# tech-srl/code2vec

Measured on NVIDIA H100. Metric: path-contexts/sec (train step, batch 1024x200), higher is better.
Workload: dtype tf32 operands / fp32 accumulate+storage

## Files before the change

### code2vec_b200/csrc/umma_gemm.cuh

```cuda
#pragma once
#include <cuda.h>
#include <cuda_runtime.h>
#include <limits.h>
#include <stdint.h>

#include "common.cuh"

namespace c2v {
namespace umma {

constexpr int BM = 128;
constexpr int BN = 128;
constexpr int BK = 32;
constexpr int WG_K = 8;
constexpr int STAGES = 4;
constexpr int kThreads = 4 * 128;
constexpr int kRegsProducer = 72;
constexpr int kRegsConsumer = 128;
constexpr int kRegsEpilogue = 184;
static_assert(kRegsProducer + 2 * kRegsConsumer + kRegsEpilogue == 4 * 128, "the roles share the CTA's registers");

__device__ __forceinline__ float fast_tanh(float x) {
  float e, r;
  asm("ex2.approx.ftz.f32 %0, %1;" : "=f"(e) : "f"(x * 2.885390081777927f));
  asm("rcp.approx.ftz.f32 %0, %1;" : "=f"(r) : "f"(e + 1.f));
  return fmaf(-2.f, r, 1.f);
}

__device__ __forceinline__ uint32_t smem_u32(const void* p) { return (uint32_t)__cvta_generic_to_shared(p); }

__device__ __forceinline__ void mbar_init(uint64_t* bar, uint32_t count) {
  asm volatile("mbarrier.init.shared::cta.b64 [%0], %1;" ::"r"(smem_u32(bar)), "r"(count));
}
__device__ __forceinline__ void mbar_expect_tx(uint64_t* bar, uint32_t bytes) {
  asm volatile("mbarrier.expect_tx.relaxed.cta.shared::cta.b64 [%0], %1;" ::"r"(smem_u32(bar)), "r"(bytes) : "memory");
}
__device__ __forceinline__ void mbar_arrive(uint64_t* bar) {
  asm volatile("mbarrier.arrive.shared::cta.b64 _, [%0];" ::"r"(smem_u32(bar)) : "memory");
}
__device__ __forceinline__ void mbar_arrive_expect_tx(uint64_t* bar, uint32_t bytes) {
  asm volatile("mbarrier.arrive.expect_tx.shared::cta.b64 _, [%0], %1;" ::"r"(smem_u32(bar)), "r"(bytes) : "memory");
}
__device__ __forceinline__ bool mbar_try_wait(uint64_t* bar, uint32_t parity) {
  uint32_t ok;
  asm volatile(
      "{\n\t.reg .pred p;\n\t"
      "mbarrier.try_wait.parity.shared::cta.b64 p, [%1], %2;\n\t"
      "selp.u32 %0, 1, 0, p;\n\t}"
      : "=r"(ok) : "r"(smem_u32(bar)), "r"(parity) : "memory");
  return ok != 0;
}
template <bool SLEEP = false>
__device__ __forceinline__ void mbar_wait(uint64_t* bar, uint32_t parity) {
  if (mbar_try_wait(bar, parity)) return;
  const long long t0 = clock64();
  uint32_t ns = 32;
  while (!mbar_try_wait(bar, parity)) {
    if (SLEEP) {
      __nanosleep(ns);
      if (ns < 256) ns *= 2;
    }
    if (clock64() - t0 > 20000000000LL) __trap();
  }
}
__device__ __forceinline__ void fence_proxy_async_smem() { asm volatile("fence.proxy.async.shared::cta;" ::: "memory"); }

__device__ __forceinline__ void tma_load_2d(void* smem_dst, const CUtensorMap* map, uint64_t* bar, int c0, int c1) {
  asm volatile(
      "cp.async.bulk.tensor.2d.shared::cluster.global.mbarrier::complete_tx::bytes [%0], [%1, {%3, %4}], [%2];"
      ::"r"(smem_u32(smem_dst)), "l"(map), "r"(smem_u32(bar)), "r"(c0), "r"(c1) : "memory");
}

__device__ __forceinline__ uint64_t gmma_desc(uint32_t saddr) {
  return (uint64_t)((saddr >> 4) & 0x3FFF) | (1ull << 16) | ((uint64_t)(1024 >> 4) << 32) | (1ull << 62);
}
__device__ __forceinline__ void wg_fence() { asm volatile("wgmma.fence.sync.aligned;" ::: "memory"); }
__device__ __forceinline__ void wg_commit() { asm volatile("wgmma.commit_group.sync.aligned;" ::: "memory"); }
template <int N>
__device__ __forceinline__ void wg_wait() { asm volatile("wgmma.wait_group.sync.aligned %0;" ::"n"(N) : "memory"); }
template <int R>
__device__ __forceinline__ void wg_regs_dec() { asm volatile("setmaxnreg.dec.sync.aligned.u32 %0;" ::"n"(R)); }
template <int R>
__device__ __forceinline__ void wg_regs_inc() { asm volatile("setmaxnreg.inc.sync.aligned.u32 %0;" ::"n"(R)); }
__device__ __forceinline__ void wgmma_tf32(float (&d)[64], uint64_t da, uint64_t db, uint32_t accumulate) {
  asm volatile(
      "{\n\t.reg .pred p;\n\t"
      "setp.ne.b32 p, %66, 0;\n\t"
      "wgmma.mma_async.sync.aligned.m64n128k8.f32.tf32.tf32 "
      "{%0, %1, %2, %3, %4, %5, %6, %7, %8, %9, %10, %11, %12, %13, %14, %15, %16, %17, %18, %19, %20, %21, %22, %23, "
      "%24, %25, %26, %27, %28, %29, %30, %31, %32, %33, %34, %35, %36, %37, %38, %39, %40, %41, %42, %43, %44, %45, "
      "%46, %47, %48, %49, %50, %51, %52, %53, %54, %55, %56, %57, %58, %59, %60, %61, %62, %63}, %64, %65, p, 1, 1;\n\t}"
      : "+f"(d[0]), "+f"(d[1]), "+f"(d[2]), "+f"(d[3]), "+f"(d[4]), "+f"(d[5]), "+f"(d[6]), "+f"(d[7]), "+f"(d[8]),
        "+f"(d[9]), "+f"(d[10]), "+f"(d[11]), "+f"(d[12]), "+f"(d[13]), "+f"(d[14]), "+f"(d[15]), "+f"(d[16]),
        "+f"(d[17]), "+f"(d[18]), "+f"(d[19]), "+f"(d[20]), "+f"(d[21]), "+f"(d[22]), "+f"(d[23]), "+f"(d[24]),
        "+f"(d[25]), "+f"(d[26]), "+f"(d[27]), "+f"(d[28]), "+f"(d[29]), "+f"(d[30]), "+f"(d[31]), "+f"(d[32]),
        "+f"(d[33]), "+f"(d[34]), "+f"(d[35]), "+f"(d[36]), "+f"(d[37]), "+f"(d[38]), "+f"(d[39]), "+f"(d[40]),
        "+f"(d[41]), "+f"(d[42]), "+f"(d[43]), "+f"(d[44]), "+f"(d[45]), "+f"(d[46]), "+f"(d[47]), "+f"(d[48]),
        "+f"(d[49]), "+f"(d[50]), "+f"(d[51]), "+f"(d[52]), "+f"(d[53]), "+f"(d[54]), "+f"(d[55]), "+f"(d[56]),
        "+f"(d[57]), "+f"(d[58]), "+f"(d[59]), "+f"(d[60]), "+f"(d[61]), "+f"(d[62]), "+f"(d[63])
      : "l"(da), "l"(db), "r"(accumulate));
}

struct EpiNoState {};

struct EpiStore {
  using State = EpiNoState;
  float* C;
  size_t ldc;
  size_t split_stride;
  __device__ __forceinline__ void begin(State&) const {}
  __device__ __forceinline__ void end(int, int, int, bool, State&) const {}
  __device__ __forceinline__ void observe(int, int, const uint32_t (&)[32], int, State&) const {}
  __device__ __forceinline__ float map(float x) const { return x; }
  __device__ __forceinline__ float* out(int split) const { return C + (size_t)split * split_stride; }
  using Pre = EpiNoState;
  static constexpr int kRowBatch = 8;
  static constexpr bool kMoveRegs = false;
  __device__ __forceinline__ void prefetch(const float*, size_t, Pre&) const {}
  __device__ __forceinline__ void store4(float* c, size_t off, float4 v, const Pre&) const { *reinterpret_cast<float4*>(c + off) = v; }
  __device__ __forceinline__ void store1(float* c, size_t off, float x) const { c[off] = x; }
};
template <bool PRECISE>
struct EpiTanhStoreT {
  using State = EpiNoState;
  float* C;
  size_t ldc;
  __device__ __forceinline__ void begin(State&) const {}
  __device__ __forceinline__ void end(int, int, int, bool, State&) const {}
  __device__ __forceinline__ void observe(int, int, const uint32_t (&)[32], int, State&) const {}
  __device__ __forceinline__ float map(float x) const { return PRECISE ? tanhf(x) : fast_tanh(x); }
  __device__ __forceinline__ float* out(int) const { return C; }
  using Pre = EpiNoState;
  static constexpr int kRowBatch = 8;
  __device__ __forceinline__ void prefetch(const float*, size_t, Pre&) const {}
  __device__ __forceinline__ void store4(float* c, size_t off, float4 v, const Pre&) const { *reinterpret_cast<float4*>(c + off) = v; }
  __device__ __forceinline__ void store1(float* c, size_t off, float x) const { c[off] = x; }
};

template <bool PRECISE>
struct EpiStoreLseT {
  struct State { float mx, sum; };
  float* C;
  size_t ldc;
  float2* partial;
  int slots;
  __device__ __forceinline__ float ex(float x) const { return PRECISE ? expf(x) : __expf(x); }
  __device__ __forceinline__ void begin(State& st) const { st.mx = -INFINITY; st.sum = 0.f; }
  __device__ __forceinline__ void end(int m, int slot, int, bool row_ok, State& st) const {
    if (row_ok) partial[(size_t)m * slots + slot] = make_float2(st.mx, st.sum);
  }
  __device__ __forceinline__ float map(float x) const { return x; }
  __device__ __forceinline__ float* out(int) const { return C; }
  using Pre = EpiNoState;
  static constexpr int kRowBatch = 8;
  __device__ __forceinline__ void prefetch(const float*, size_t, Pre&) const {}
  __device__ __forceinline__ void store4(float* c, size_t off, float4 v, const Pre&) const { *reinterpret_cast<float4*>(c + off) = v; }
  __device__ __forceinline__ void store1(float* c, size_t off, float x) const { c[off] = x; }
  __device__ __forceinline__ void observe(int, int, const uint32_t (&r)[32], int nvalid, State& st) const {
    float cm = -INFINITY;
    if (nvalid >= 32) {
#pragma unroll
      for (int j = 0; j < 32; ++j) cm = fmaxf(cm, __uint_as_float(r[j]));
    } else {
#pragma unroll
      for (int j = 0; j < 32; ++j)
        if (j < nvalid) cm = fmaxf(cm, __uint_as_float(r[j]));
    }
    if (cm > st.mx) { st.sum *= ex(st.mx - cm); st.mx = cm; }
    float a0 = 0.f, a1 = 0.f, a2 = 0.f, a3 = 0.f;
    if (!PRECISE && nvalid >= 32) {
      constexpr float L2E = 1.4426950408889634f;
      const float c = -st.mx * L2E;
      auto e2 = [](float t) { float y; asm("ex2.approx.ftz.f32 %0, %1;" : "=f"(y) : "f"(t)); return y; };
#pragma unroll
      for (int j = 0; j < 32; j += 4) {
        a0 += e2(fmaf(__uint_as_float(r[j + 0]), L2E, c));
        a1 += e2(fmaf(__uint_as_float(r[j + 1]), L2E, c));
        a2 += e2(fmaf(__uint_as_float(r[j + 2]), L2E, c));
        a3 += e2(fmaf(__uint_as_float(r[j + 3]), L2E, c));
      }
    } else {
#pragma unroll
      for (int j = 0; j < 32; j += 4) {
        if (j + 0 < nvalid) a0 += ex(__uint_as_float(r[j + 0]) - st.mx);
        if (j + 1 < nvalid) a1 += ex(__uint_as_float(r[j + 1]) - st.mx);
        if (j + 2 < nvalid) a2 += ex(__uint_as_float(r[j + 2]) - st.mx);
        if (j + 3 < nvalid) a3 += ex(__uint_as_float(r[j + 3]) - st.mx);
      }
    }
    st.sum += (a0 + a1) + (a2 + a3);
  }
};

template <bool PRECISE>
struct EpiLseOnlyT : EpiStoreLseT<PRECISE> {
  static constexpr bool kStores = false;
};
constexpr int kTopkEpiMax = 16;
template <bool PRECISE, bool LSE>
struct EpiTopkT : EpiStoreLseT<PRECISE> {
  using Lse = EpiStoreLseT<PRECISE>;
  struct State {
    float v[kTopkEpiMax];
    int i[kTopkEpiMax];
    typename Lse::State ls;
  };
  float* cand_val;
  int32_t* cand_idx;
  int k;
  int row0;
  static constexpr bool kStores = false;
  __device__ __forceinline__ void begin(State& st) const {
#pragma unroll
    for (int q = 0; q < kTopkEpiMax; ++q) {
      st.v[q] = q < kTopkEpiMax - k ? INFINITY : -INFINITY;
      st.i[q] = INT_MAX;
    }
    if (LSE) Lse::begin(st.ls);
  }
  __device__ __forceinline__ void insert(float x, int col, State& st) const {
#pragma unroll
    for (int q = kTopkEpiMax - 1; q > 0; --q) {
      const bool here = x > st.v[q], above = x > st.v[q - 1];
      st.v[q] = above ? st.v[q - 1] : (here ? x : st.v[q]);
      st.i[q] = above ? st.i[q - 1] : (here ? col : st.i[q]);
    }
    if (x > st.v[0]) { st.v[0] = x; st.i[0] = col; }
  }
  __device__ __forceinline__ void observe(int m, int n, const uint32_t (&r)[32], int nvalid, State& st) const {
    if (LSE) Lse::observe(m, n, r, nvalid, st.ls);
    const float kth = st.v[kTopkEpiMax - 1];
    float x[32];
    uint32_t todo = 0;
#pragma unroll
    for (int j = 0; j < 32; ++j) {
      x[j] = __uint_as_float(r[j]);
      if (j < nvalid && x[j] > kth) todo |= 1u << j;
    }
#pragma unroll 1
    while (todo) {
      const int j = __ffs(todo) - 1;
      todo &= todo - 1;
      insert(x[j], n + j, st);
    }
  }
  __device__ __forceinline__ void end(int m, int slot, int sp, bool row_ok, State& st) const {
    if (!row_ok) return;
    if (LSE) Lse::end(m, slot, sp, row_ok, st.ls);
    const size_t base = ((size_t)m * this->slots + slot) * k;
#pragma unroll
    for (int q = 0; q < kTopkEpiMax; ++q) {
      const int p = q - (kTopkEpiMax - k);
      if (p >= 0) {
        cand_val[base + p] = st.v[q];
        cand_idx[base + p] = st.i[q] == INT_MAX ? INT_MAX : st.i[q] + row0;
      }
    }
  }
};
template <bool PRECISE, bool SPLIT>
struct EpiSoftmaxGradT {
  struct State { float l; int tgt; };
  float* C;
  float* C_lo;
  size_t ldc;
  const float* lse;
  const int32_t* target;
  int row0;
  float inv_batch;
  int M;
  __device__ __forceinline__ void begin(State& st) const { st.l = 0.f; st.tgt = -1; }
  __device__ __forceinline__ void end(int, int, int, bool, State&) const {}
  __device__ __forceinline__ void observe(int m, int, const uint32_t (&)[32], int, State& st) const {
    st.l = PRECISE ? lse[m] : fmaf(-lse[m], 1.4426950408889634f, log2f(inv_batch));
    st.tgt = target[m] - row0;
  }
  __device__ __forceinline__ float map(float x) const { return x; }
  __device__ __forceinline__ float map_at(float x, int col, const State& st) const {
    float p;
    if (PRECISE) {
      p = expf(x - st.l) * inv_batch;
    } else {
      asm("ex2.approx.ftz.f32 %0, %1;" : "=f"(p) : "f"(fmaf(x, 1.4426950408889634f, st.l)));
    }
    return col == st.tgt ? p - inv_batch : p;
  }
  __device__ __forceinline__ float* out(int) const { return C; }
  using Pre = EpiNoState;
  static constexpr int kRowBatch = 8;
  __device__ __forceinline__ void prefetch(const float*, size_t, Pre&) const {}
  __device__ __forceinline__ void store4(float* c, size_t off, float4 v, const Pre&) const {
    if (SPLIT) {
      float4 hi, lo;
      split_tf32(v, hi, lo);
      *reinterpret_cast<float4*>(c + off) = hi;
      *reinterpret_cast<float4*>(C_lo + off) = lo;
    } else {
      *reinterpret_cast<float4*>(c + off) = v;
    }
  }
  __device__ __forceinline__ void store1(float* c, size_t off, float x) const {
    if (SPLIT) {
      float hi, lo;
      split_tf32(x, hi, lo);
      c[off] = hi; C_lo[off] = lo;
    } else {
      c[off] = x;
    }
  }
};

template <bool PRECISE, bool SPLIT>
struct EpiExpSumT {
  struct State { float mx, sum; };
  float* C;
  float* C_lo;
  size_t ldc;
  const float* offset;
  float2* partial;
  int slots;
  __device__ __forceinline__ void begin(State& st) const { st.mx = 0.f; st.sum = 0.f; }
  __device__ __forceinline__ void end(int m, int slot, int, bool row_ok, State& st) const {
    if (row_ok) partial[(size_t)m * slots + slot] = make_float2(st.mx, st.sum);
  }
  __device__ __forceinline__ float map(float x) const { return x; }
  __device__ __forceinline__ float* out(int) const { return C; }
  using Pre = EpiNoState;
  static constexpr int kRowBatch = 8;
  __device__ __forceinline__ void prefetch(const float*, size_t, Pre&) const {}
  __device__ __forceinline__ void store4(float* c, size_t off, float4 v, const Pre&) const {
    if (SPLIT) {
      float4 hi, lo;
      split_tf32(v, hi, lo);
      *reinterpret_cast<float4*>(c + off) = hi;
      *reinterpret_cast<float4*>(C_lo + off) = lo;
    } else {
      *reinterpret_cast<float4*>(c + off) = v;
    }
  }
  __device__ __forceinline__ void store1(float* c, size_t off, float x) const {
    if (SPLIT) {
      float hi, lo;
      split_tf32(x, hi, lo);
      c[off] = hi; C_lo[off] = lo;
    } else {
      c[off] = x;
    }
  }
  __device__ __forceinline__ void observe(int m, int, uint32_t (&r)[32], int nvalid, State& st) const {
    const float c = offset[m];
    float a0 = 0.f, a1 = 0.f, a2 = 0.f, a3 = 0.f, x0 = 0.f, x1 = 0.f, x2 = 0.f, x3 = 0.f;
    if (!PRECISE && nvalid >= 32) {
      constexpr float L2E = 1.4426950408889634f;
      const float c2 = -c * L2E;
      auto e2 = [](float t) { float y; asm("ex2.approx.ftz.f32 %0, %1;" : "=f"(y) : "f"(t)); return y; };
#pragma unroll
      for (int j = 0; j < 32; j += 4) {
        const float u0 = e2(fmaf(__uint_as_float(r[j + 0]), L2E, c2)), u1 = e2(fmaf(__uint_as_float(r[j + 1]), L2E, c2));
        const float u2 = e2(fmaf(__uint_as_float(r[j + 2]), L2E, c2)), u3 = e2(fmaf(__uint_as_float(r[j + 3]), L2E, c2));
        r[j + 0] = __float_as_uint(u0); r[j + 1] = __float_as_uint(u1); r[j + 2] = __float_as_uint(u2); r[j + 3] = __float_as_uint(u3);
        a0 += u0; a1 += u1; a2 += u2; a3 += u3;
        x0 = fmaxf(x0, u0); x1 = fmaxf(x1, u1); x2 = fmaxf(x2, u2); x3 = fmaxf(x3, u3);
      }
    } else {
#pragma unroll
      for (int j = 0; j < 32; ++j) {
        float u = 0.f;
        if (j < nvalid) u = PRECISE ? expf(__uint_as_float(r[j]) - c) : __expf(__uint_as_float(r[j]) - c);
        r[j] = __float_as_uint(u);
        if ((j & 3) == 0) { a0 += u; x0 = fmaxf(x0, u); }
        else if ((j & 3) == 1) { a1 += u; x1 = fmaxf(x1, u); }
        else if ((j & 3) == 2) { a2 += u; x2 = fmaxf(x2, u); }
        else { a3 += u; x3 = fmaxf(x3, u); }
      }
    }
    st.sum += (a0 + a1) + (a2 + a3);
    st.mx = fmaxf(st.mx, fmaxf(fmaxf(x0, x1), fmaxf(x2, x3)));
  }
};
template <bool PRECISE>
struct EpiStoreLseGatedT : EpiStoreLseT<PRECISE> {
  const int* gate;
};

using EpiTanhStore = EpiTanhStoreT<false>;
using EpiTanhStorePrecise = EpiTanhStoreT<true>;
using EpiStoreLse = EpiStoreLseT<false>;
using EpiStoreLsePrecise = EpiStoreLseT<true>;

struct EpiAdam {
  using State = EpiNoState;
  float* P;
  float* Mo;
  float* Vo;
  size_t ldc;
  float lr_t, b1, b2, eps, omb1, omb2;
  int l2_prefetch;
  __device__ __forceinline__ void begin(State&) const {}
  __device__ __forceinline__ void end(int, int, int, bool, State&) const {}
  __device__ __forceinline__ void observe(int, int, const uint32_t (&)[32], int, State&) const {}
  __device__ __forceinline__ float map(float x) const { return x; }
  __device__ __forceinline__ float* out(int) const { return P; }
  __device__ __forceinline__ void upd(float& pp, float gg, float& mm, float& vv) const {
    mm = __fadd_rn(__fmul_rn(mm, b1), __fmul_rn(omb1, gg));
    vv = __fadd_rn(__fmul_rn(vv, b2), __fmul_rn(omb2, __fmul_rn(gg, gg)));
    pp = adam_move_dense(pp, lr_t, mm, vv, eps);
  }
  __device__ __forceinline__ void prefetch_tile(int m, int n0, int ncols, int M, int N) const {
    if (m >= M || !l2_prefetch) return;
    const size_t row = (size_t)m * ldc;
    for (int n = n0; n < n0 + ncols && n < N; n += 32) {
      asm volatile("prefetch.global.L2 [%0];" ::"l"(P + row + n));
      asm volatile("prefetch.global.L2 [%0];" ::"l"(Mo + row + n));
      asm volatile("prefetch.global.L2 [%0];" ::"l"(Vo + row + n));
    }
  }
  struct Pre { float4 p, m, v; };
  static constexpr int kRowBatch = 4;
  __device__ __forceinline__ void prefetch(const float* c, size_t off, Pre& q) const {
    q.p = *reinterpret_cast<const float4*>(c + off);
    q.m = *reinterpret_cast<const float4*>(Mo + off);
    q.v = *reinterpret_cast<const float4*>(Vo + off);
  }
  __device__ __forceinline__ void store4(float* c, size_t off, float4 g, const Pre& q) const {
    float4 p = q.p, m = q.m, v = q.v;
    upd(p.x, g.x, m.x, v.x); upd(p.y, g.y, m.y, v.y); upd(p.z, g.z, m.z, v.z); upd(p.w, g.w, m.w, v.w);
    *reinterpret_cast<float4*>(c + off) = p;
    *reinterpret_cast<float4*>(Mo + off) = m;
    *reinterpret_cast<float4*>(Vo + off) = v;
  }
  __device__ __forceinline__ void store1(float* c, size_t off, float g) const {
    float p = c[off], m = Mo[off], v = Vo[off];
    upd(p, g, m, v);
    c[off] = p; Mo[off] = m; Vo[off] = v;
  }
};

template <class Epi>
__device__ __forceinline__ auto epi_map(const Epi& epi, float x, int col, const typename Epi::State& st, int)
    -> decltype(epi.map_at(x, col, st)) {
  return epi.map_at(x, col, st);
}
template <class Epi>
__device__ __forceinline__ float epi_map(const Epi& epi, float x, int, const typename Epi::State&, long) {
  return epi.map(x);
}
template <class Epi>
__device__ __forceinline__ auto epi_gate_closed(const Epi& epi, int) -> decltype(*epi.gate == 0) { return *epi.gate == 0; }
template <class Epi>
__device__ __forceinline__ bool epi_gate_closed(const Epi&, long) { return false; }
template <class Epi>
__device__ __forceinline__ auto epi_prefetch_tile(const Epi& epi, int m, int n0, int ncols, int M, int N, int)
    -> decltype(epi.prefetch_tile(m, n0, ncols, M, N)) {
  epi.prefetch_tile(m, n0, ncols, M, N);
}
template <class Epi>
__device__ __forceinline__ void epi_prefetch_tile(const Epi&, int, int, int, int, int, long) {}
template <class Epi>
constexpr bool epi_move_regs(...) { return true; }
template <class Epi, bool V = Epi::kMoveRegs>
constexpr bool epi_move_regs(int) { return V; }
template <class Epi>
constexpr bool epi_stores(...) { return true; }
template <class Epi, bool V = Epi::kStores>
constexpr bool epi_stores(int) { return V; }

template <class Epi>
__device__ __forceinline__ void store_chunk(const Epi& epi, const typename Epi::State& est, const uint32_t (&r)[32], float* stage, int lane,
                                            int m_base, int n, int M, int N, float* cbase, size_t ldc) {
#pragma unroll
  for (int j4 = 0; j4 < 8; ++j4) {
    const int pos = j4 ^ (lane & 7);
    *reinterpret_cast<float4*>(stage + lane * 32 + pos * 4) =
        make_float4(epi_map(epi, __uint_as_float(r[4 * j4]), n + 4 * j4, est, 0), epi_map(epi, __uint_as_float(r[4 * j4 + 1]), n + 4 * j4 + 1, est, 0),
                    epi_map(epi, __uint_as_float(r[4 * j4 + 2]), n + 4 * j4 + 2, est, 0), epi_map(epi, __uint_as_float(r[4 * j4 + 3]), n + 4 * j4 + 3, est, 0));
  }
  __syncwarp();
  const int col4 = lane & 7;
  const int gn = n + col4 * 4;
  constexpr int kBatch = Epi::kRowBatch;
  static_assert(8 % kBatch == 0, "the batches tile the chunk's 8 row groups: a remainder would reach into the next block");
#pragma unroll
  for (int it0 = 0; it0 < 8; it0 += kBatch) {
    float4 v[kBatch];
    typename Epi::Pre pre[kBatch];
#pragma unroll
    for (int i = 0; i < kBatch; ++i) {
      const int row = (it0 + i) * 4 + (lane >> 3);
      v[i] = *reinterpret_cast<const float4*>(stage + row * 32 + ((col4 ^ (row & 7)) * 4));
      const int gm = m_base + row;
      if (gm < M && gn + 3 < N) epi.prefetch(cbase, (size_t)gm * ldc + gn, pre[i]);
    }
#pragma unroll
    for (int i = 0; i < kBatch; ++i) {
      const int gm = m_base + (it0 + i) * 4 + (lane >> 3);
      if (gm < M && gn < N) {
        const size_t off = (size_t)gm * ldc + gn;
        if (gn + 3 < N) {
          epi.store4(cbase, off, v[i], pre[i]);
        } else {
          epi.store1(cbase, off, v[i].x);
          if (gn + 1 < N) epi.store1(cbase, off + 1, v[i].y);
          if (gn + 2 < N) epi.store1(cbase, off + 2, v[i].z);
        }
      }
    }
  }
  __syncwarp();
}

struct AXNone {
  static constexpr int kKind = 0;
};

struct SoftmaxGradArgs {
  const float* lse;
  const int32_t* target;
  int row0;
  float inv_batch;
};
__device__ __forceinline__ float ex2_approx(float x) {
  float y;
  asm("ex2.approx.ftz.f32 %0, %1;" : "=f"(y) : "f"(x));
  return y;
}
constexpr float kLog2e = 1.4426950408889634f;

template <bool EX_IS_M>
struct AXSoftmaxGrad {
  static constexpr int kKind = 1;
  SoftmaxGradArgs a;
  __device__ __forceinline__ void example(int ex, float& c, int& tgt) const {
    c = fmaf(-a.lse[ex], kLog2e, log2f(a.inv_batch));
    tgt = a.target[ex] - a.row0;
  }
  __device__ __forceinline__ float p(float s, int y, float c, int tgt) const {
    return ex2_approx(fmaf(s, kLog2e, c)) - ((y == tgt) ? a.inv_batch : 0.f);
  }
  __device__ __forceinline__ float4 xform(float4 v, int x, int k, int X, int K) const {
    static_assert(EX_IS_M, "the MN-major tile is transformed element by element as it is transposed (umma_gemm_kernel)");
    if (x >= X) return v;
    float c;
    int tgt;
    example(x, c, tgt);
    float e[4] = {v.x, v.y, v.z, v.w};
#pragma unroll
    for (int j = 0; j < 4; ++j) e[j] = (k + j < K) ? p(e[j], k + j, c, tgt) : 0.f;
    return make_float4(e[0], e[1], e[2], e[3]);
  }
};

struct AXGather {
  static constexpr int kKind = 2;
  ContextSource cs;
  Dropout dp;
  float* Xout;
};

__device__ __forceinline__ float4 ld4(const float* p) { return __ldg(reinterpret_cast<const float4*>(p)); }

template <class AX>
__device__ __forceinline__ void load_tile_k(uint8_t* dst, const float* base, size_t ld, int x0, int X, int k0, int K, int t,
                                            const AX& ax) {
  const int c = t & 7, rg = t >> 3, k = k0 + c * 4;
  float4 v[8];
#pragma unroll
  for (int i = 0; i < 8; ++i) {
    const int x = x0 + rg + 16 * i;
    v[i] = make_float4(0.f, 0.f, 0.f, 0.f);
    if (x < X) {
      const float* p = base + (size_t)x * ld + k;
      if (k + 3 < K) {
        v[i] = ld4(p);
      } else {
        if (k < K) v[i].x = p[0];
        if (k + 1 < K) v[i].y = p[1];
        if (k + 2 < K) v[i].z = p[2];
      }
    }
  }
#pragma unroll
  for (int i = 0; i < 8; ++i) {
    const int r = rg + 16 * i;
    if constexpr (AX::kKind == 1) v[i] = ax.xform(v[i], x0 + r, k, X, K);
    *reinterpret_cast<float4*>(dst + r * 128 + ((c ^ (r & 7)) << 4)) = v[i];
  }
}

template <class F>
__device__ __forceinline__ void transpose_box(uint8_t* box, int lane, const F& f) {
  const uint32_t rd = smem_u32(box) + lane * 4, wr = (smem_u32(box) + lane * 128) ^ ((lane & 7) << 4);
  float v[BK];
#pragma unroll
  for (int k = 0; k < BK; ++k) {
    asm volatile("ld.shared.f32 %0, [%1];" : "=f"(v[k]) : "r"((rd ^ ((k & 7) << 4)) + k * 128) : "memory");
    v[k] = f(v[k], k);
  }
  __syncwarp();
#pragma unroll
  for (int c = 0; c < BK / 4; ++c)
    asm volatile("st.shared.v4.f32 [%0], {%1, %2, %3, %4};" ::"r"(wr ^ (c << 4)), "f"(v[4 * c]), "f"(v[4 * c + 1]), "f"(v[4 * c + 2]),
                 "f"(v[4 * c + 3]) : "memory");
}

__device__ __forceinline__ void load_tile_gather(uint8_t* dst, const AXGather& g, int m0, int M, int kb, bool write_x, int t) {
  const int c = t & 7, rg = t >> 3;
  const int kps = g.cs.d / BK, seg = kb / kps;
  const int col = (kb - seg * kps) * BK + c * 4;
  const int32_t* ids = seg == 0 ? g.cs.src : seg == 1 ? g.cs.pth : g.cs.tgt;
  const int K = 3 * g.cs.d;
  float4 v[8];
#pragma unroll
  for (int i = 0; i < 8; ++i) {
    const int m = m0 + rg + 16 * i;
    v[i] = make_float4(0.f, 0.f, 0.f, 0.f);
    if (m < M) v[i] = ld4(((seg == 1) ? table_row(g.cs.path, ids[m], g.cs.d) : table_row(g.cs.tok, ids[m], g.cs.d)) + col);
  }
#pragma unroll
  for (int i = 0; i < 8; ++i) {
    const int r = rg + 16 * i, m = m0 + r;
    if (g.dp.enabled) {
      const float4 mlt = dropout_mult4(g.dp, m, kb * (BK / 4) + c);
      v[i].x *= mlt.x; v[i].y *= mlt.y; v[i].z *= mlt.z; v[i].w *= mlt.w;
    }
    *reinterpret_cast<float4*>(dst + r * 128 + ((c ^ (r & 7)) << 4)) = v[i];
    if (write_x && m < M) *reinterpret_cast<float4*>(g.Xout + (size_t)m * K + kb * BK + c * 4) = v[i];
  }
}

struct GemmShape {
  int M, N, K;
  int m_tiles, n_tiles, splits;
  int kblocks_per_split;
  int n_fastest;
  int terms;
};
struct GemmPtrs {
  const float* a;
  size_t lda;
};

struct SmemLayout {
  static constexpr int kABytes = BM * BK * 4;
  static constexpr int kBBytes = BN * BK * 4;
  static constexpr int kStageBytes = kABytes + kBBytes;
  static constexpr int kEpiOffset = STAGES * kStageBytes;
  static constexpr int kEpiBytes = 64 * BN * 4;
  static constexpr int kBarOffset = kEpiOffset + 2 * kEpiBytes;
  static constexpr int kTotal = kBarOffset + 256 + 1024;
  static_assert((3 * STAGES + 2) * 8 <= 256, "the barriers fit their block");
  static_assert(kTotal <= 232448, "exceeds the 227 KB of shared memory a CTA can opt into");
};

template <bool A_MN, bool B_MN, class Epi, class AX = AXNone>
__global__ void __launch_bounds__(kThreads, 1)
umma_gemm_kernel(const __grid_constant__ CUtensorMap tmA, const __grid_constant__ CUtensorMap tmB,
                 const __grid_constant__ CUtensorMap tmAlo, const __grid_constant__ CUtensorMap tmBlo, GemmShape gs,
                 GemmPtrs ptr, Epi epi, AX ax = AX{}) {
  if (epi_gate_closed(epi, 0)) return;
  using L = SmemLayout;
  static_assert(!(A_MN && AX::kKind == 2), "the gathered A tile is K-major");
  constexpr bool kTmaA = !A_MN && AX::kKind == 0;
  constexpr bool kTmaB = !B_MN;
  constexpr uint32_t kTxBytes = (kTmaA ? L::kABytes : 0) + (kTmaB ? L::kBBytes : 0);
  constexpr uint32_t kMnTxBytes = (A_MN ? L::kABytes : 0) + (B_MN ? L::kBBytes : 0);
  constexpr int kLag = kMnTxBytes ? STAGES - 2 : 0;
  static_assert(kLag <= STAGES - 2, "the producer would wait for a stage only a step it has not published can free");
  extern __shared__ uint8_t smem_raw[];
  uint8_t* smem = reinterpret_cast<uint8_t*>((reinterpret_cast<uintptr_t>(smem_raw) + 1023) & ~(uintptr_t)1023);
  uint64_t* full_bar = reinterpret_cast<uint64_t*>(smem + L::kBarOffset);
  uint64_t* empty_bar = full_bar + STAGES;
  uint64_t* landed_bar = empty_bar + STAGES;
  uint64_t* epi_full = landed_bar + STAGES;
  uint64_t* epi_empty = epi_full + 1;

  const int wg = threadIdx.x >> 7, warp = threadIdx.x >> 5, lane = threadIdx.x & 31;
  const int total_items = gs.m_tiles * gs.n_tiles * gs.splits;
  const int total_kblocks = (gs.K + BK - 1) / BK;

  if (threadIdx.x == 0) {
    for (int s = 0; s < STAGES; ++s) { mbar_init(&full_bar[s], 128); mbar_init(&empty_bar[s], 8); mbar_init(&landed_bar[s], 1); }
    mbar_init(epi_full, 256);
    mbar_init(epi_empty, 128);
    asm volatile("fence.mbarrier_init.release.cluster;" ::: "memory");
  }
  __syncthreads();

  auto decode = [&](int item, int& mt, int& nt, int& sp) {
    if (gs.n_fastest) {
      nt = item % gs.n_tiles;
      const int r = item / gs.n_tiles;
      mt = r % gs.m_tiles;
      sp = r / gs.m_tiles;
    } else {
      mt = item % gs.m_tiles;
      const int r = item / gs.m_tiles;
      nt = r % gs.n_tiles;
      sp = r / gs.n_tiles;
    }
  };

  if (wg == 0) {
    if constexpr (epi_move_regs<Epi>(0)) wg_regs_dec<kRegsProducer>();
    const int t = threadIdx.x;
    struct Cursor {
      int item, mt, nt, kb, kb0, kb1, pass;
      int stage;
      uint32_t phase;
    };
    auto seek = [&](Cursor& c) {
      for (; c.item < total_items; c.item += gridDim.x) {
        int sp;
        decode(c.item, c.mt, c.nt, sp);
        c.kb = c.kb0 = sp * gs.kblocks_per_split;
        c.kb1 = min(total_kblocks, c.kb0 + gs.kblocks_per_split);
        c.pass = gs.terms == 3 ? 0 : 2;
        if (c.kb0 < c.kb1) return;
      }
    };
    auto next = [&](Cursor& c) {
      if (++c.stage == STAGES) { c.stage = 0; c.phase ^= 1; }
      if (++c.kb < c.kb1) return;
      if (c.pass < 2) { ++c.pass; c.kb = c.kb0; return; }
      c.item += gridDim.x;
      seek(c);
    };
    auto issue = [&](const Cursor& c) {
      mbar_wait(&empty_bar[c.stage], c.phase ^ 1);
      uint8_t* sa = smem + c.stage * L::kStageBytes;
      uint8_t* sb = sa + L::kABytes;
      const int k0 = c.kb * BK;
      const bool a_lo = c.pass == 0, b_lo = c.pass == 1;
      if (t == 0) {
        if (kTxBytes) {
          mbar_expect_tx(&full_bar[c.stage], kTxBytes);
          if (kTmaA) tma_load_2d(sa, a_lo ? &tmAlo : &tmA, &full_bar[c.stage], k0, c.mt * BM);
          if (kTmaB) tma_load_2d(sb, b_lo ? &tmBlo : &tmB, &full_bar[c.stage], k0, c.nt * BN);
        }
        if (kMnTxBytes) {
          mbar_arrive_expect_tx(&landed_bar[c.stage], kMnTxBytes);
#pragma unroll
          for (int q = 0; q < 4; ++q) {
            if (A_MN) tma_load_2d(sa + q * 4096, a_lo ? &tmAlo : &tmA, &landed_bar[c.stage], c.mt * BM + 32 * q, k0);
            if (B_MN) tma_load_2d(sb + q * 4096, b_lo ? &tmBlo : &tmB, &landed_bar[c.stage], c.nt * BN + 32 * q, k0);
          }
        }
      }
      if constexpr (AX::kKind == 2) load_tile_gather(sa, ax, c.mt * BM, gs.M, c.kb, ax.Xout != nullptr && c.nt == 0, t);
      else if constexpr (!A_MN && !kTmaA) load_tile_k(sa, ptr.a, ptr.lda, c.mt * BM, gs.M, k0, gs.K, t, ax);
    };
    auto complete = [&](const Cursor& c) {
      uint8_t* sa = smem + c.stage * L::kStageBytes;
      uint8_t* sb = sa + L::kABytes;
      if constexpr (kMnTxBytes != 0) {
        if constexpr (A_MN && AX::kKind == 1) {
          const int k0 = c.kb * BK, x = c.mt * BM + 32 * warp + lane;
          float ce = 0.f;
          int te = -1;
          if (k0 + lane < gs.K) ax.example(k0 + lane, ce, te);
          mbar_wait(&landed_bar[c.stage], c.phase);
          transpose_box(sa + warp * 4096, lane, [&](float s, int k) {
            const float ck = __shfl_sync(0xffffffffu, ce, k);
            const int tk = __shfl_sync(0xffffffffu, te, k);
            return (x < gs.M && k0 + k < gs.K) ? ax.p(s, x, ck, tk) : 0.f;
          });
        } else {
          mbar_wait(&landed_bar[c.stage], c.phase);
          if constexpr (A_MN) transpose_box(sa + warp * 4096, lane, [](float s, int) { return s; });
        }
        if constexpr (B_MN) transpose_box(sb + warp * 4096, lane, [](float s, int) { return s; });
      }
      if constexpr (!kTmaA || !kTmaB) fence_proxy_async_smem();
      mbar_arrive(&full_bar[c.stage]);
    };
    Cursor ld{static_cast<int>(blockIdx.x), 0, 0, 0, 0, 0, 0, 0, 0u};
    seek(ld);
    if constexpr (kLag == 0) {
      for (; ld.item < total_items; next(ld)) { issue(ld); complete(ld); }
    } else {
      Cursor tr = ld;
      for (int ahead = 0; tr.item < total_items;) {
        const bool more = ld.item < total_items;
        if (more) { issue(ld); next(ld); ++ahead; }
        if (ahead > kLag || !more) { complete(tr); next(tr); --ahead; }
      }
    }
  } else if (wg <= 2) {
    const int cw = wg - 1, wl = warp & 3;
    const int g = lane >> 2;
    const uint32_t stg_row = smem_u32(smem + L::kEpiOffset + cw * L::kEpiBytes) + (wl >> 1) * 4096 + (16 * (wl & 1) + g) * 128 +
                             ((g ^ ((lane >> 1) & 1)) << 4) + 8 * (lane & 1);
    int stage = 0;
    uint32_t phase = 0, epi_phase = 0;
    float acc[64];
    for (int item = blockIdx.x; item < total_items; item += gridDim.x, epi_phase ^= 1) {
      int mt, nt, sp;
      decode(item, mt, nt, sp);
      const int kb0 = sp * gs.kblocks_per_split;
      const int kb1 = min(total_kblocks, kb0 + gs.kblocks_per_split);
      const int n_steps = (kb1 - kb0) * gs.terms;
      int prev = 0;
      for (int it = 0; it < n_steps; ++it) {
        mbar_wait(&full_bar[stage], phase);
        const uint32_t sa = smem_u32(smem + stage * L::kStageBytes) + cw * 64 * 128;
        const uint32_t sb = smem_u32(smem + stage * L::kStageBytes + L::kABytes);
        wg_fence();
#pragma unroll
        for (int k = 0; k < BK / WG_K; ++k)
          wgmma_tf32(acc, gmma_desc(sa + k * WG_K * 4), gmma_desc(sb + k * WG_K * 4), (it > 0 || k > 0) ? 1u : 0u);
        wg_commit();
        wg_wait<1>();
        if (it > 0 && lane == 0) mbar_arrive(&empty_bar[prev]);
        prev = stage;
        if (++stage == STAGES) { stage = 0; phase ^= 1; }
      }
      wg_wait<0>();
      if (n_steps > 0 && lane == 0) mbar_arrive(&empty_bar[prev]);

      mbar_wait(epi_empty, epi_phase ^ 1);
#pragma unroll
      for (int j = 0; j < BN / 8; ++j) {
#pragma unroll
        for (int i = 0; i < 2; ++i)
          asm volatile("st.shared.v2.f32 [%0], {%1, %2};" ::"r"((stg_row ^ ((j & 3) << 5)) + 8192 * (j >> 2) + 1024 * i),
                       "f"(acc[4 * j + 2 * i]), "f"(acc[4 * j + 2 * i + 1]) : "memory");
      }
      mbar_arrive(epi_full);
    }
  } else {
    if constexpr (epi_move_regs<Epi>(0)) wg_regs_inc<kRegsEpilogue>();
    const int w = warp & 3;
    float* stg = reinterpret_cast<float*>(smem + L::kEpiOffset + (w >> 1) * L::kEpiBytes);
    auto prefetch_item = [&](int it) {
      if (it >= total_items) return;
      int mt2, nt2, sp2;
      decode(it, mt2, nt2, sp2);
      epi_prefetch_tile(epi, mt2 * BM + 32 * w + lane, nt2 * BN, BN, gs.M, gs.N, 0);
    };
    prefetch_item(blockIdx.x);
    uint32_t epi_phase = 0;
    for (int item = blockIdx.x; item < total_items; item += gridDim.x, epi_phase ^= 1) {
      int mt, nt, sp;
      decode(item, mt, nt, sp);
      prefetch_item(item + gridDim.x);
      mbar_wait<true>(epi_full, epi_phase);
      const int m_base = mt * BM + 32 * w, m = m_base + lane;
      float* cbase = epi.out(sp);
#pragma unroll 1
      for (int p = 0; p < 2; ++p) {
        typename Epi::State est;
        epi.begin(est);
#pragma unroll 1
        for (int q = p; q < 4; q += 2) {
          float* blk = stg + ((w & 1) | (q << 1)) * 1024;
          uint32_t r[32];
#pragma unroll
          for (int c4 = 0; c4 < 8; ++c4) {
            const float4 x = *reinterpret_cast<const float4*>(blk + lane * 32 + ((c4 ^ (lane & 7)) << 2));
            r[4 * c4] = __float_as_uint(x.x); r[4 * c4 + 1] = __float_as_uint(x.y);
            r[4 * c4 + 2] = __float_as_uint(x.z); r[4 * c4 + 3] = __float_as_uint(x.w);
          }
          __syncwarp();
          const int n = nt * BN + 32 * q;
          if (n < gs.N) {
            if (m < gs.M) epi.observe(m, n, r, gs.N - n, est);
            if (epi_stores<Epi>(0)) store_chunk(epi, est, r, blk, lane, m_base, n, gs.M, gs.N, cbase, epi.ldc);
          }
        }
        epi.end(m, 2 * nt + p, sp, m < gs.M, est);
      }
      mbar_arrive(epi_empty);
    }
  }
}

typedef CUresult (*EncodeTiledFn)(CUtensorMap*, CUtensorMapDataType, cuuint32_t, void*, const cuuint64_t*, const cuuint64_t*,
                                  const cuuint32_t*, const cuuint32_t*, CUtensorMapInterleave, CUtensorMapSwizzle,
                                  CUtensorMapL2promotion, CUtensorMapFloatOOBfill);

inline EncodeTiledFn get_encode_fn() {
  static EncodeTiledFn fn = nullptr;
  if (!fn) {
    void* p = nullptr;
    cudaDriverEntryPointQueryResult qres;
    if (cudaGetDriverEntryPoint("cuTensorMapEncodeTiled", &p, cudaEnableDefault, &qres) == cudaSuccess && p)
      fn = reinterpret_cast<EncodeTiledFn>(p);
  }
  return fn;
}

struct TensorMapKey {
  const float* base;
  uint64_t rows, cols, ld;
  uint32_t box_rows;
  bool operator==(const TensorMapKey& o) const {
    return base == o.base && rows == o.rows && cols == o.cols && ld == o.ld && box_rows == o.box_rows;
  }
};
struct TensorMapCache {
  static constexpr int kCap = 96;
  TensorMapKey key[kCap];
  CUtensorMap map[kCap];
  int n = 0, next = 0;
};
inline bool make_tensor_map(CUtensorMap* map, const float* base, uint64_t rows, uint64_t cols, uint64_t ld, uint32_t box_rows) {
  static thread_local TensorMapCache cache;
  const TensorMapKey k{base, rows, cols, ld, box_rows};
  for (int i = 0; i < cache.n; ++i)
    if (cache.key[i] == k) { *map = cache.map[i]; return true; }
  EncodeTiledFn fn = get_encode_fn();
  if (!fn) return false;
  cuuint64_t dims[2] = {cols, rows};
  cuuint64_t strides[1] = {ld * sizeof(float)};
  cuuint32_t box[2] = {32, box_rows};
  cuuint32_t estr[2] = {1, 1};
  CUresult r = fn(map, CU_TENSOR_MAP_DATA_TYPE_FLOAT32, 2, const_cast<float*>(base), dims, strides, box, estr,
                  CU_TENSOR_MAP_INTERLEAVE_NONE, CU_TENSOR_MAP_SWIZZLE_128B, CU_TENSOR_MAP_L2_PROMOTION_L2_256B,
                  CU_TENSOR_MAP_FLOAT_OOB_FILL_NONE);
  if (r != CUDA_SUCCESS) return false;
  const int slot = (cache.n < TensorMapCache::kCap) ? cache.n++ : (cache.next++ % TensorMapCache::kCap);
  cache.key[slot] = k;
  cache.map[slot] = *map;
  return true;
}

struct Operand {
  const float* base;
  size_t ld;
  bool major_mn;
  const float* lo = nullptr;
};

inline bool operand_map(CUtensorMap* map, const float* base, bool major_mn, int X, int K, size_t ld) {
  return major_mn ? make_tensor_map(map, base, (uint64_t)K, (uint64_t)X, ld, BK) : make_tensor_map(map, base, (uint64_t)X, (uint64_t)K, ld, BM);
}

inline GemmShape make_shape(int M, int N, int K, int splits, int terms) {
  GemmShape gs;
  gs.M = M; gs.N = N; gs.K = K;
  gs.terms = terms;
  gs.m_tiles = (M + BM - 1) / BM;
  gs.n_tiles = (N + BN - 1) / BN;
  const int total_kblocks = (K + BK - 1) / BK;
  if (splits < 1) splits = 1;
  if (splits > total_kblocks) splits = total_kblocks;
  gs.kblocks_per_split = (total_kblocks + splits - 1) / splits;
  gs.splits = (total_kblocks + gs.kblocks_per_split - 1) / gs.kblocks_per_split;
  gs.n_fastest = (gs.n_tiles < gs.m_tiles) ? 1 : 0;
  return gs;
}

template <bool A_MN, bool B_MN, class Epi, class AX>
inline cudaError_t launch_kernel(cudaStream_t st, const CUtensorMap& tmA, const CUtensorMap& tmB, const CUtensorMap& tmAlo,
                                 const CUtensorMap& tmBlo, const GemmShape& gs, const GemmPtrs& ptr, const Epi& epi, int num_sms,
                                 const AX& ax) {
  auto kern = umma_gemm_kernel<A_MN, B_MN, Epi, AX>;
  cudaError_t e = cudaFuncSetAttribute(kern, cudaFuncAttributeMaxDynamicSharedMemorySize, SmemLayout::kTotal);
  if (e != cudaSuccess) return e;
  int grid = gs.m_tiles * gs.n_tiles * gs.splits;
  if (grid > num_sms) grid = num_sms;
  kern<<<grid, kThreads, SmemLayout::kTotal, st>>>(tmA, tmB, tmAlo, tmBlo, gs, ptr, epi, ax);
  return cudaGetLastError();
}

template <bool A_MN, bool B_MN, class Epi, class AX = AXNone>
inline cudaError_t launch_cfg(cudaStream_t st, int M, int N, int K, int splits, const Operand& A, const Operand& B, const Epi& epi,
                              int num_sms, const AX& ax = AX{}) {
  CUtensorMap tmA{}, tmB{}, tmAlo{}, tmBlo{};
  const bool three = A.lo != nullptr && B.lo != nullptr;
  if ((A.lo != nullptr) != (B.lo != nullptr)) return cudaErrorInvalidValue;
  if (AX::kKind != 0 && three) return cudaErrorInvalidValue;
  if (A_MN || AX::kKind == 0) {
    if (!operand_map(&tmA, A.base, A_MN, M, K, A.ld)) return cudaErrorInvalidValue;
    if (three && !operand_map(&tmAlo, A.lo, A_MN, M, K, A.ld)) return cudaErrorInvalidValue;
  }
  if (!operand_map(&tmB, B.base, B_MN, N, K, B.ld)) return cudaErrorInvalidValue;
  if (three && !operand_map(&tmBlo, B.lo, B_MN, N, K, B.ld)) return cudaErrorInvalidValue;
  const GemmPtrs ptr{A.base, A.ld};
  return launch_kernel<A_MN, B_MN, Epi, AX>(st, tmA, tmB, tmAlo, tmBlo, make_shape(M, N, K, splits, three ? 3 : 1), ptr, epi,
                                            num_sms, ax);
}

inline int effective_splits(int K, int splits) {
  const int total_kblocks = (K + BK - 1) / BK;
  if (splits < 1) splits = 1;
  if (splits > total_kblocks) splits = total_kblocks;
  const int per = (total_kblocks + splits - 1) / splits;
  return (total_kblocks + per - 1) / per;
}

inline int lse_slots(int n) { return 2 * ((n + BN - 1) / BN); }

template <class Epi>
inline cudaError_t launch(cudaStream_t st, int M, int N, int K, int splits, const Operand& A, const Operand& B, const Epi& epi,
                          int num_sms) {
  if (!A.major_mn && !B.major_mn) return launch_cfg<false, false, Epi>(st, M, N, K, splits, A, B, epi, num_sms);
  if (!A.major_mn && B.major_mn) return launch_cfg<false, true, Epi>(st, M, N, K, splits, A, B, epi, num_sms);
  if (A.major_mn && !B.major_mn) return launch_cfg<true, false, Epi>(st, M, N, K, splits, A, B, epi, num_sms);
  return launch_cfg<true, true, Epi>(st, M, N, K, splits, A, B, epi, num_sms);
}

template <class Epi>
inline cudaError_t launch_ctx_fused(cudaStream_t st, int M, int N, const float* W, size_t ldw, const ContextSource& cs,
                                    const Dropout& dp, float* Xout, const Epi& epi, int num_sms) {
  const int K = 3 * cs.d;
  GemmShape gs = make_shape(M, N, K, 1, 1);
  gs.n_fastest = 1;
  const CUtensorMap none{};
  CUtensorMap tmW{};
  if (!operand_map(&tmW, W, true, N, K, ldw)) return cudaErrorInvalidValue;
  return launch_kernel<false, true, Epi, AXGather>(st, none, tmW, none, none, gs, GemmPtrs{nullptr, 0}, epi, num_sms, AXGather{cs, dp, Xout});
}

inline bool operand_ok(const Operand& o) {
  return (reinterpret_cast<uintptr_t>(o.base) % 16 == 0) && (o.ld % 4 == 0);
}

}
}
```

Measured before the change: 30.92 million.

## Feed MN-major A operand to wgmma from registers instead of producer transpose

For GEMMs whose A tile is MN-major, the producer no longer transposes A in shared memory. It TMA-loads the boxes directly, and the consumer warpgroups read A fragments into registers, apply the softmax-gradient transform there, and issue register-sourced wgmma with double-buffered fragments. Register budgets per role are now templated, giving consumers more registers and the producer fewer when A is MN-major. This removes the producer's transpose and shared-memory round trip from the critical path, but adds shared-memory loads, shuffles and register pressure on the consumers, and changes the epilogue staging row mapping.

```diff
diff --git a/code2vec_b200/csrc/umma_gemm.cuh b/code2vec_b200/csrc/umma_gemm.cuh
--- a/code2vec_b200/csrc/umma_gemm.cuh
+++ b/code2vec_b200/csrc/umma_gemm.cuh
@@ -15,10 +15,13 @@
 constexpr int WG_K = 8;
 constexpr int STAGES = 4;
 constexpr int kThreads = 4 * 128;
-constexpr int kRegsProducer = 72;
-constexpr int kRegsConsumer = 128;
-constexpr int kRegsEpilogue = 184;
-static_assert(kRegsProducer + 2 * kRegsConsumer + kRegsEpilogue == 4 * 128, "the roles share the CTA's registers");
+template <bool A_MN, bool B_MN>
+struct Regs {
+  static constexpr int kProducer = (A_MN && !B_MN) ? 40 : 72;
+  static constexpr int kConsumer = A_MN ? 144 : 128;
+  static constexpr int kEpilogue = 4 * 128 - kProducer - 2 * kConsumer;
+  static_assert(kEpilogue >= 128, "the epilogue never gives registers up");
+};
 
 __device__ __forceinline__ float fast_tanh(float x) {
   float e, r;
@@ -100,6 +103,25 @@
         "+f"(d[57]), "+f"(d[58]), "+f"(d[59]), "+f"(d[60]), "+f"(d[61]), "+f"(d[62]), "+f"(d[63])
       : "l"(da), "l"(db), "r"(accumulate));
 }
+__device__ __forceinline__ void wgmma_tf32_rs(float (&d)[64], const uint32_t* a, uint64_t db, uint32_t accumulate) {
+  asm volatile(
+      "{\n\t.reg .pred p;\n\t"
+      "setp.ne.b32 p, %69, 0;\n\t"
+      "wgmma.mma_async.sync.aligned.m64n128k8.f32.tf32.tf32 "
+      "{%0, %1, %2, %3, %4, %5, %6, %7, %8, %9, %10, %11, %12, %13, %14, %15, %16, %17, %18, %19, %20, %21, %22, %23, "
+      "%24, %25, %26, %27, %28, %29, %30, %31, %32, %33, %34, %35, %36, %37, %38, %39, %40, %41, %42, %43, %44, %45, "
+      "%46, %47, %48, %49, %50, %51, %52, %53, %54, %55, %56, %57, %58, %59, %60, %61, %62, %63}, {%64, %65, %66, %67}, "
+      "%68, p, 1, 1;\n\t}"
+      : "+f"(d[0]), "+f"(d[1]), "+f"(d[2]), "+f"(d[3]), "+f"(d[4]), "+f"(d[5]), "+f"(d[6]), "+f"(d[7]), "+f"(d[8]),
+        "+f"(d[9]), "+f"(d[10]), "+f"(d[11]), "+f"(d[12]), "+f"(d[13]), "+f"(d[14]), "+f"(d[15]), "+f"(d[16]),
+        "+f"(d[17]), "+f"(d[18]), "+f"(d[19]), "+f"(d[20]), "+f"(d[21]), "+f"(d[22]), "+f"(d[23]), "+f"(d[24]),
+        "+f"(d[25]), "+f"(d[26]), "+f"(d[27]), "+f"(d[28]), "+f"(d[29]), "+f"(d[30]), "+f"(d[31]), "+f"(d[32]),
+        "+f"(d[33]), "+f"(d[34]), "+f"(d[35]), "+f"(d[36]), "+f"(d[37]), "+f"(d[38]), "+f"(d[39]), "+f"(d[40]),
+        "+f"(d[41]), "+f"(d[42]), "+f"(d[43]), "+f"(d[44]), "+f"(d[45]), "+f"(d[46]), "+f"(d[47]), "+f"(d[48]),
+        "+f"(d[49]), "+f"(d[50]), "+f"(d[51]), "+f"(d[52]), "+f"(d[53]), "+f"(d[54]), "+f"(d[55]), "+f"(d[56]),
+        "+f"(d[57]), "+f"(d[58]), "+f"(d[59]), "+f"(d[60]), "+f"(d[61]), "+f"(d[62]), "+f"(d[63])
+      : "r"(a[0]), "r"(a[1]), "r"(a[2]), "r"(a[3]), "l"(db), "r"(accumulate));
+}
 
 struct EpiNoState {};
 
@@ -538,7 +560,7 @@
     return ex2_approx(fmaf(s, kLog2e, c)) - ((y == tgt) ? a.inv_batch : 0.f);
   }
   __device__ __forceinline__ float4 xform(float4 v, int x, int k, int X, int K) const {
-    static_assert(EX_IS_M, "the MN-major tile is transformed element by element as it is transposed (umma_gemm_kernel)");
+    static_assert(EX_IS_M, "the MN-major tile is transformed in the consumers' A fragments (umma_gemm_kernel)");
     if (x >= X) return v;
     float c;
     int tgt;
@@ -587,21 +609,20 @@
   }
 }
 
-template <class F>
-__device__ __forceinline__ void transpose_box(uint8_t* box, int lane, const F& f) {
+__device__ __forceinline__ void transpose_box(uint8_t* box, int lane) {
   const uint32_t rd = smem_u32(box) + lane * 4, wr = (smem_u32(box) + lane * 128) ^ ((lane & 7) << 4);
   float v[BK];
 #pragma unroll
-  for (int k = 0; k < BK; ++k) {
+  for (int k = 0; k < BK; ++k)
     asm volatile("ld.shared.f32 %0, [%1];" : "=f"(v[k]) : "r"((rd ^ ((k & 7) << 4)) + k * 128) : "memory");
-    v[k] = f(v[k], k);
-  }
   __syncwarp();
 #pragma unroll
   for (int c = 0; c < BK / 4; ++c)
     asm volatile("st.shared.v4.f32 [%0], {%1, %2, %3, %4};" ::"r"(wr ^ (c << 4)), "f"(v[4 * c]), "f"(v[4 * c + 1]), "f"(v[4 * c + 2]),
                  "f"(v[4 * c + 3]) : "memory");
 }
+
+__device__ __forceinline__ int rs_row(int w, int g, int i) { return 32 * (w >> 1) + 16 * (g >> 2) + 8 * (w & 1) + 4 * i + (g & 3); }
 
 __device__ __forceinline__ void load_tile_gather(uint8_t* dst, const AXGather& g, int m0, int M, int kb, bool write_x, int t) {
   const int c = t & 7, rg = t >> 3;
@@ -660,10 +681,11 @@
   if (epi_gate_closed(epi, 0)) return;
   using L = SmemLayout;
   static_assert(!(A_MN && AX::kKind == 2), "the gathered A tile is K-major");
-  constexpr bool kTmaA = !A_MN && AX::kKind == 0;
+  using R = Regs<A_MN, B_MN>;
+  constexpr bool kTmaA = A_MN || AX::kKind == 0;
   constexpr bool kTmaB = !B_MN;
   constexpr uint32_t kTxBytes = (kTmaA ? L::kABytes : 0) + (kTmaB ? L::kBBytes : 0);
-  constexpr uint32_t kMnTxBytes = (A_MN ? L::kABytes : 0) + (B_MN ? L::kBBytes : 0);
+  constexpr uint32_t kMnTxBytes = B_MN ? L::kBBytes : 0;
   constexpr int kLag = kMnTxBytes ? STAGES - 2 : 0;
   static_assert(kLag <= STAGES - 2, "the producer would wait for a stage only a step it has not published can free");
   extern __shared__ uint8_t smem_raw[];
@@ -701,7 +723,7 @@
   };
 
   if (wg == 0) {
-    if constexpr (epi_move_regs<Epi>(0)) wg_regs_dec<kRegsProducer>();
+    if constexpr (epi_move_regs<Epi>(0)) wg_regs_dec<R::kProducer>();
     const int t = threadIdx.x;
     struct Cursor {
       int item, mt, nt, kb, kb0, kb1, pass;
@@ -734,41 +756,27 @@
       if (t == 0) {
         if (kTxBytes) {
           mbar_expect_tx(&full_bar[c.stage], kTxBytes);
-          if (kTmaA) tma_load_2d(sa, a_lo ? &tmAlo : &tmA, &full_bar[c.stage], k0, c.mt * BM);
+          if (kTmaA && A_MN) {
+#pragma unroll
+            for (int q = 0; q < 4; ++q) tma_load_2d(sa + q * 4096, a_lo ? &tmAlo : &tmA, &full_bar[c.stage], c.mt * BM + 32 * q, k0);
+          } else if (kTmaA) {
+            tma_load_2d(sa, a_lo ? &tmAlo : &tmA, &full_bar[c.stage], k0, c.mt * BM);
+          }
           if (kTmaB) tma_load_2d(sb, b_lo ? &tmBlo : &tmB, &full_bar[c.stage], k0, c.nt * BN);
         }
         if (kMnTxBytes) {
           mbar_arrive_expect_tx(&landed_bar[c.stage], kMnTxBytes);
 #pragma unroll
-          for (int q = 0; q < 4; ++q) {
-            if (A_MN) tma_load_2d(sa + q * 4096, a_lo ? &tmAlo : &tmA, &landed_bar[c.stage], c.mt * BM + 32 * q, k0);
-            if (B_MN) tma_load_2d(sb + q * 4096, b_lo ? &tmBlo : &tmB, &landed_bar[c.stage], c.nt * BN + 32 * q, k0);
-          }
+          for (int q = 0; q < 4; ++q) tma_load_2d(sb + q * 4096, b_lo ? &tmBlo : &tmB, &landed_bar[c.stage], c.nt * BN + 32 * q, k0);
         }
       }
       if constexpr (AX::kKind == 2) load_tile_gather(sa, ax, c.mt * BM, gs.M, c.kb, ax.Xout != nullptr && c.nt == 0, t);
-      else if constexpr (!A_MN && !kTmaA) load_tile_k(sa, ptr.a, ptr.lda, c.mt * BM, gs.M, k0, gs.K, t, ax);
+      else if constexpr (!kTmaA) load_tile_k(sa, ptr.a, ptr.lda, c.mt * BM, gs.M, k0, gs.K, t, ax);
     };
     auto complete = [&](const Cursor& c) {
-      uint8_t* sa = smem + c.stage * L::kStageBytes;
-      uint8_t* sb = sa + L::kABytes;
-      if constexpr (kMnTxBytes != 0) {
-        if constexpr (A_MN && AX::kKind == 1) {
-          const int k0 = c.kb * BK, x = c.mt * BM + 32 * warp + lane;
-          float ce = 0.f;
-          int te = -1;
-          if (k0 + lane < gs.K) ax.example(k0 + lane, ce, te);
-          mbar_wait(&landed_bar[c.stage], c.phase);
-          transpose_box(sa + warp * 4096, lane, [&](float s, int k) {
-            const float ck = __shfl_sync(0xffffffffu, ce, k);
-            const int tk = __shfl_sync(0xffffffffu, te, k);
-            return (x < gs.M && k0 + k < gs.K) ? ax.p(s, x, ck, tk) : 0.f;
-          });
-        } else {
-          mbar_wait(&landed_bar[c.stage], c.phase);
-          if constexpr (A_MN) transpose_box(sa + warp * 4096, lane, [](float s, int) { return s; });
-        }
-        if constexpr (B_MN) transpose_box(sb + warp * 4096, lane, [](float s, int) { return s; });
+      if constexpr (B_MN) {
+        mbar_wait(&landed_bar[c.stage], c.phase);
+        transpose_box(smem + c.stage * L::kStageBytes + L::kABytes + warp * 4096, lane);
       }
       if constexpr (!kTmaA || !kTmaB) fence_proxy_async_smem();
       mbar_arrive(&full_bar[c.stage]);
@@ -786,10 +794,23 @@
       }
     }
   } else if (wg <= 2) {
+    if constexpr (A_MN && epi_move_regs<Epi>(0)) wg_regs_inc<R::kConsumer>();
     const int cw = wg - 1, wl = warp & 3;
     const int g = lane >> 2;
-    const uint32_t stg_row = smem_u32(smem + L::kEpiOffset + cw * L::kEpiBytes) + (wl >> 1) * 4096 + (16 * (wl & 1) + g) * 128 +
-                             ((g ^ ((lane >> 1) & 1)) << 4) + 8 * (lane & 1);
+    const uint32_t stg_base = smem_u32(smem + L::kEpiOffset + cw * L::kEpiBytes);
+    const uint32_t stg_row = stg_base + (wl >> 1) * 4096 + (16 * (wl & 1) + g) * 128 + ((g ^ ((lane >> 1) & 1)) << 4) + 8 * (lane & 1);
+    uint32_t stg_rs[2], a_frag[2][2];
+    if constexpr (A_MN) {
+      const int t = lane & 3;
+#pragma unroll
+      for (int i = 0; i < 2; ++i) {
+        const int r = rs_row(wl, g, i), x = r & 31;
+        stg_rs[i] = stg_base + (r >> 5) * 4096 + x * 128 + ((((lane >> 1) & 1) ^ (r & 7)) << 4) + 8 * (lane & 1);
+#pragma unroll
+        for (int c = 0; c < 2; ++c)
+          a_frag[i][c] = (2 * cw + (wl >> 1)) * 4096 + 128 * (t + 4 * c) + ((4 * x) ^ ((t + 4 * c) << 4));
+      }
+    }
     int stage = 0;
     uint32_t phase = 0, epi_phase = 0;
     float acc[64];
@@ -800,19 +821,66 @@
       const int kb1 = min(total_kblocks, kb0 + gs.kblocks_per_split);
       const int n_steps = (kb1 - kb0) * gs.terms;
       int prev = 0;
-      for (int it = 0; it < n_steps; ++it) {
-        mbar_wait(&full_bar[stage], phase);
-        const uint32_t sa = smem_u32(smem + stage * L::kStageBytes) + cw * 64 * 128;
-        const uint32_t sb = smem_u32(smem + stage * L::kStageBytes + L::kABytes);
-        wg_fence();
-#pragma unroll
-        for (int k = 0; k < BK / WG_K; ++k)
-          wgmma_tf32(acc, gmma_desc(sa + k * WG_K * 4), gmma_desc(sb + k * WG_K * 4), (it > 0 || k > 0) ? 1u : 0u);
-        wg_commit();
-        wg_wait<1>();
-        if (it > 0 && lane == 0) mbar_arrive(&empty_bar[prev]);
-        prev = stage;
-        if (++stage == STAGES) { stage = 0; phase ^= 1; }
+      if constexpr (!A_MN) {
+        for (int it = 0; it < n_steps; ++it) {
+          mbar_wait(&full_bar[stage], phase);
+          const uint32_t sa = smem_u32(smem + stage * L::kStageBytes) + cw * 64 * 128;
+          const uint32_t sb = smem_u32(smem + stage * L::kStageBytes + L::kABytes);
+          wg_fence();
+#pragma unroll
+          for (int k = 0; k < BK / WG_K; ++k)
+            wgmma_tf32(acc, gmma_desc(sa + k * WG_K * 4), gmma_desc(sb + k * WG_K * 4), (it > 0 || k > 0) ? 1u : 0u);
+          wg_commit();
+          wg_wait<1>();
+          if (it > 0 && lane == 0) mbar_arrive(&empty_bar[prev]);
+          prev = stage;
+          if (++stage == STAGES) { stage = 0; phase ^= 1; }
+        }
+      } else {
+        const int x_tile = mt * BM + 64 * cw;
+        auto load_a = [&](uint32_t (&a)[16], int it) {
+          float ce = 0.f;
+          int te = -1;
+          const int k0 = (kb0 + it) * BK;
+          if constexpr (AX::kKind == 1)
+            if (k0 + lane < gs.K) ax.example(k0 + lane, ce, te);
+          mbar_wait(&full_bar[stage], phase);
+          const uint32_t sa = smem_u32(smem + stage * L::kStageBytes);
+#pragma unroll
+          for (int kk = 0; kk < BK / WG_K; ++kk)
+#pragma unroll
+            for (int c = 0; c < 2; ++c)
+#pragma unroll
+              for (int i = 0; i < 2; ++i) {
+                uint32_t& v = a[4 * kk + 2 * c + i];
+                asm volatile("ld.shared.b32 %0, [%1];" : "=r"(v) : "r"(sa + a_frag[i][c] + 1024 * kk) : "memory");
+                if constexpr (AX::kKind == 1) {
+                  const int k = WG_K * kk + (lane & 3) + 4 * c, x = x_tile + rs_row(wl, g, i);
+                  const float ck = __shfl_sync(0xffffffffu, ce, k);
+                  const int tk = __shfl_sync(0xffffffffu, te, k);
+                  v = __float_as_uint((x < gs.M && k0 + k < gs.K) ? ax.p(__uint_as_float(v), x, ck, tk) : 0.f);
+                }
+                v &= 0xffffe000u;
+              }
+        };
+        auto step = [&](const uint32_t (&a)[16], uint32_t (&a_next)[16], int it) {
+          const uint32_t sb = smem_u32(smem + stage * L::kStageBytes + L::kABytes);
+          wg_fence();
+#pragma unroll
+          for (int k = 0; k < BK / WG_K; ++k) wgmma_tf32_rs(acc, a + 4 * k, gmma_desc(sb + k * WG_K * 4), (it > 0 || k > 0) ? 1u : 0u);
+          wg_commit();
+          wg_wait<1>();
+          if (it > 0 && lane == 0) mbar_arrive(&empty_bar[prev]);
+          prev = stage;
+          if (++stage == STAGES) { stage = 0; phase ^= 1; }
+          if (it + 1 < n_steps) load_a(a_next, it + 1);
+        };
+        uint32_t fa[16], fb[16];
+        if (n_steps > 0) load_a(fa, 0);
+        for (int it = 0; it < n_steps; it += 2) {
+          step(fa, fb, it);
+          if (it + 1 < n_steps) step(fb, fa, it + 1);
+        }
       }
       wg_wait<0>();
       if (n_steps > 0 && lane == 0) mbar_arrive(&empty_bar[prev]);
@@ -822,13 +890,14 @@
       for (int j = 0; j < BN / 8; ++j) {
 #pragma unroll
         for (int i = 0; i < 2; ++i)
-          asm volatile("st.shared.v2.f32 [%0], {%1, %2};" ::"r"((stg_row ^ ((j & 3) << 5)) + 8192 * (j >> 2) + 1024 * i),
+          asm volatile("st.shared.v2.f32 [%0], {%1, %2};" ::"r"(A_MN ? (stg_rs[i] ^ ((j & 3) << 5)) + 8192 * (j >> 2)
+                                                                   : (stg_row ^ ((j & 3) << 5)) + 8192 * (j >> 2) + 1024 * i),
                        "f"(acc[4 * j + 2 * i]), "f"(acc[4 * j + 2 * i + 1]) : "memory");
       }
       mbar_arrive(epi_full);
     }
   } else {
-    if constexpr (epi_move_regs<Epi>(0)) wg_regs_inc<kRegsEpilogue>();
+    if constexpr (epi_move_regs<Epi>(0)) wg_regs_inc<R::kEpilogue>();
     const int w = warp & 3;
     float* stg = reinterpret_cast<float*>(smem + L::kEpiOffset + (w >> 1) * L::kEpiBytes);
     auto prefetch_item = [&](int it) {
```

Measured after the change: 31.23 million (median of 6 runs). 1.01x the previous value.
